# ligengen/EgoGen

Hardware: AMD Instinct MI355X
Metric: PPO env-steps/sec (512 parallel SMPL-X agents) (higher is better)
Workload: dtype f32 (blend GEMM: shape/template columns as 2-term bf16 splits, pose correctives as one fp16 product, fp32 accumulate); PPO update products on 2-term bf16 splits; rollout policy layers on 2-term bf16 splits

## Files before the change

### egogen_amd/csrc/body_model.hip

```cpp
#include <algorithm>
#include <atomic>
#include <cstdlib>

#include "lbs_pack.h"

static thread_local hipEvent_t g_prof_start = nullptr, g_prof_stop = nullptr;
extern "C" int egx_profile_next_lbs(void* start_event, void* stop_event) {
  g_prof_start = static_cast<hipEvent_t>(start_event);
  g_prof_stop = static_cast<hipEvent_t>(stop_event);
  return EGX_OK;
}

namespace {
constexpr int BODY_PAD = 256;
}

__global__ void egx_gather_kernel(const float* __restrict__ picked, int B, int NP, int M,
                                  const int* __restrict__ marker_slot, const int* __restrict__ extra_slot,
                                  const int* __restrict__ lmk_slot, const float* __restrict__ lmk_bary,
                                  float* __restrict__ out_joints, float* __restrict__ out_markers) {
  const int b = blockIdx.x;
  const float* pk = picked + (size_t)b * NP * 3;
  for (int i = threadIdx.x; i < M + NEXTRA + NLMK; i += blockDim.x) {
    if (i < M) {
      if (out_markers) {
        const float* s = pk + marker_slot[i] * 3;
        float* o = out_markers + ((size_t)b * M + i) * 3;
        o[0] = s[0]; o[1] = s[1]; o[2] = s[2];
      }
    } else if (out_joints) {
      float* o = out_joints + ((size_t)b * EGX_NUM_JOINTS_OUT + NJ + (i - M)) * 3;
      if (i < M + NEXTRA) {
        const float* s = pk + extra_slot[i - M] * 3;
        o[0] = s[0]; o[1] = s[1]; o[2] = s[2];
      } else {
        const int l = i - M - NEXTRA;
        float acc[3] = {0.f, 0.f, 0.f};
        for (int k = 0; k < 3; ++k) {
          const float* s = pk + lmk_slot[l * 3 + k] * 3;
          const float w = lmk_bary[l * 3 + k];
          acc[0] += s[0] * w; acc[1] += s[1] * w; acc[2] += s[2] * w;
        }
        o[0] = acc[0]; o[1] = acc[1]; o[2] = acc[2];
      }
    }
  }
}

extern "C" int egx_body_model_create(const egx_body_model_host* d, egx_body_model** out) {
  EGX_REQUIRE(d && out, "null argument");
  LbsPacked p;
  if (int rc = lbs_pack_model(d, &p)) return rc;
  auto* m = new egx_body_model();
  static_cast<LbsModelDims&>(*m) = p;
  auto u16 = [](bf16x8** dptr) { return reinterpret_cast<unsigned short**>(dptr); };
  int rc = EGX_OK;
  if ((rc = egx_upload(&m->cull_E, p.cull_E)) || (rc = egx_upload(&m->cull_D0, p.cull_D0)) || (rc = egx_upload(u16(&m->dirs3), p.dirs3)) ||
      (rc = egx_upload(u16(&m->dirs4), p.dirs4)) || (rc = egx_upload(u16(&m->skinW), p.skinW)) || (rc = egx_upload(&m->skin_ks_off, p.skin_ks_off)) ||
      (rc = egx_upload(&m->dirs_rm, p.dirs_rm)) || (rc = egx_upload(&m->vorig, p.perm)) || (rc = egx_upload(&m->pick_tiles, p.pick_tiles)) ||
      (rc = egx_upload(&m->sdf_tiles, p.sdf_tiles)) || (rc = egx_upload(&m->dirs, p.dirs)) || (rc = egx_upload(&m->tj_off, p.tj_off)) ||
      (rc = egx_upload(&m->tj_idx, p.tj_idx)) || (rc = egx_upload(&m->tj_w, p.tj_w)) || (rc = egx_upload(&m->pick_slot, p.pick_slot)) ||
      (rc = egx_upload(&m->vflags, p.vflags)) || (rc = egx_upload(&m->pc, p.pc)) || (rc = egx_upload(&m->marker_slot, p.marker_slot)) ||
      (rc = egx_upload(&m->extra_slot, p.extra_slot)) || (rc = egx_upload(&m->lmk_slot, p.lmk_slot)) ||
      (rc = egx_upload(&m->lmk_bary, p.lmk_bary))) {
    egx_body_model_destroy(m);
    return rc;
  }
  *out = m;
  return EGX_OK;
}

extern "C" void egx_body_model_destroy(egx_body_model* m) {
  if (!m) return;
  (void)hipFree(m->dirs); (void)hipFree(m->dirs3); (void)hipFree(m->dirs4); (void)hipFree(m->tj_off); (void)hipFree(m->tj_idx); (void)hipFree(m->tj_w);
  (void)hipFree(m->pick_slot); (void)hipFree(m->pick_tiles); (void)hipFree(m->sdf_tiles); (void)hipFree(m->vflags); (void)hipFree(m->vorig); (void)hipFree(m->pc); (void)hipFree(m->marker_slot);
  (void)hipFree(m->extra_slot); (void)hipFree(m->lmk_slot); (void)hipFree(m->lmk_bary);
  (void)hipFree(m->cull_E); (void)hipFree(m->cull_D0);
  (void)hipFree(m->skinW); (void)hipFree(m->skin_ks_off); (void)hipFree(m->dirs_rm);
  delete m;
}

extern "C" int egx_body_model_num_verts(const egx_body_model* m) { return m ? m->V : 0; }
extern "C" int egx_body_model_nnz(const egx_body_model* m) { return m ? m->NW : 0; }
extern "C" int egx_body_model_lbs_vertices(const egx_body_model* m, int with_sdf) {
  return m ? (with_sdf ? m->verts_sdf_tiles : m->verts_pick_tiles) : 0;
}

namespace {
template <typename Parse>
int switch_value(std::atomic<int>& g, const char* env_name, Parse&& parse) {
  int v = g.load();
  if (v < 0) {
    const char* e = getenv(env_name);
    v = parse(std::string(e ? e : ""));
    if (v >= 0) g.store(v);
  }
  return v;
}
std::atomic<int> g_blend_mode{-1};
int blend_mode() {
  return switch_value(g_blend_mode, "EGX_LBS_BLEND", [](const std::string& v) {
    return (v == "f32" || v == "0") ? 0 : ((v == "bf16x3" || v == "1") ? 1 : ((v == "bf16x2" || v == "2") ? 2 : ((v.empty() || v == "f16mix" || v == "3") ? 3 : -2)));
  });
}
std::atomic<int> g_cull{-1};
int culling_on() {
  return switch_value(g_cull, "EGX_LBS_CULL", [](const std::string& v) { return v == "1" ? 1 : 0; });
}
std::atomic<int> g_wave_tile{-1};
int wave_tile() {
  return switch_value(g_wave_tile, "EGX_LBS_WAVE_TILE", [](const std::string& v) { return atoi(v.c_str()); });
}
std::atomic<int> g_fixq_cap{0};

struct WsLayout {
  size_t feat, feat4, A4, picked, total;
  size_t fvec, jpos, order, flags, items, counts;
  size_t fix_e, fix_stats;
  size_t skinB, cinit;
  size_t fixq;
  size_t Bp;
  int items_stride;
};
WsLayout ws_layout(const egx_body_model* m, int B) {
  const size_t Bp = egx_align_up((size_t)B, BODY_PAD);
  WsLayout w;
  w.Bp = Bp;
// ... 253 lines not shown
```

### egogen_amd/csrc/env.hip

```cpp
#include "egx_common.h"
#include "egx_frame.h"
#include "egx_reward.h"

namespace {

constexpr int NT = 20, THIS = 2, NM = 67, NJO = EGX_NUM_JOINTS_OUT, SD = 402, XB = EGX_XB_DIM;
constexpr int NRAY = 32;
constexpr int BLK = 128;

__device__ __forceinline__ float block_reduce(float v, float* sh, int op ) {
  sh[threadIdx.x] = v;
  __syncthreads();
  for (int s = BLK / 2; s > 0; s >>= 1) {
    if ((int)threadIdx.x < s) {
      const float a = sh[threadIdx.x], b = sh[threadIdx.x + s];
      sh[threadIdx.x] = op == 0 ? a + b : (op == 1 ? fminf(a, b) : fmaxf(a, b));
    }
    __syncthreads();
  }
  const float r = sh[0];
  __syncthreads();
  return r;
}

struct SceneDev {
  const float* edges;
  const int* edge_off;
  const float* tris;
  const int* tri_off;
  const float* floor_h;
  const float* map_lin;
  int map_res;
  float* crowd_bbox;
  int crowd_G, crowd_S, crowd_k;
  float crowd_half;
  int crowd_polygon;
  int crowd_static;
};

__device__ __forceinline__ bool point_in_rings(const float* edges, int e0, int e1, double x, double y) {
  int crossings = 0;
  for (int e = e0; e < e1; ++e) {
    const float* q = edges + (size_t)e * 4;
    const double x0 = q[0], y0 = q[1], x1 = q[2], y1 = q[3];
    if ((y0 > y) != (y1 > y)) {
      const double xint = x0 + (y - y0) * (x1 - x0) / (y1 - y0);
      if (x < xint) ++crossings;
    }
  }
  return (crossings & 1) == 1;
}

__device__ __forceinline__ int scene_num_edges(const SceneDev& sc, int sc_i) {
  if (sc.crowd_bbox)
    return (sc.crowd_polygon ? sc.edge_off[1] - sc.edge_off[0] : 4) + (sc.crowd_static ? 0 : 4 * (sc.crowd_G - 1));
  return sc.edge_off[sc_i + 1] - sc.edge_off[sc_i];
}
__device__ __forceinline__ void scene_edge(const SceneDev& sc, int sc_i, int e, double& x0, double& y0, double& x1, double& y1) {
  if (!sc.crowd_bbox) {
    const float* p = sc.edges + (size_t)(sc.edge_off[sc_i] + e) * 4;
    x0 = p[0]; y0 = p[1]; x1 = p[2]; y1 = p[3];
    return;
  }
  const int n_ext = sc.crowd_polygon ? sc.edge_off[1] - sc.edge_off[0] : 4;
  if (sc.crowd_polygon && e < n_ext) {
    const float* p = sc.edges + (size_t)(sc.edge_off[0] + e) * 4;
    x0 = p[0]; y0 = p[1]; x1 = p[2]; y1 = p[3];
    return;
  }
  float lo[2], hi[2];
  int q;
  if (e < n_ext) {
    lo[0] = lo[1] = -sc.crowd_half; hi[0] = hi[1] = sc.crowd_half;
    q = e;
  } else {
    e -= n_ext - 4;
    int other = (e - 4) >> 2;
    if (other >= sc.crowd_k) ++other;
    const float* b = sc.crowd_bbox + ((size_t)other * sc.crowd_S + sc_i) * 4;
    lo[0] = b[0]; lo[1] = b[1]; hi[0] = b[2]; hi[1] = b[3];
    q = (e - 4) & 3;
  }
  const double cx[4] = {lo[0], hi[0], hi[0], lo[0]}, cy[4] = {lo[1], lo[1], hi[1], hi[1]};
  x0 = cx[q]; y0 = cy[q]; x1 = cx[(q + 1) & 3]; y1 = cy[(q + 1) & 3];
}

__device__ void egosensing_frame(const SceneDev& sc, int scene, const float* j23, const float* j24, const float* j56,
                                 const float* j57, double ray_len, float* out32 , int tid, int nthreads) {
  const float lx = j57[0] - j23[0] + j56[0] - j24[0];
  const float ly = j57[1] - j23[1] + j56[1] - j24[1];
  double la0 = (double)lx, la1 = (double)ly;
  const double ln = sqrt(la0 * la0 + la1 * la1);
  la0 /= ln; la1 /= ln;
  const float exf = (j23[0] + j24[0]) / 2.f, eyf = (j23[1] + j24[1]) / 2.f;
  const double ox = (double)exf, oy = (double)eyf;
  const int ne = scene_num_edges(sc, scene);
  int crossings = 0;
  for (int e = 0; e < ne; ++e) {
    double x0, y0, x1, y1;
    scene_edge(sc, scene, e, x0, y0, x1, y1);
    if ((y0 > oy) != (y1 > oy)) {
      const double xint = x0 + (oy - y0) * (x1 - x0) / (y1 - y0);
// ... 81 lines not shown

struct EnvCfg {
  float reproj_factor, goal_thresh, pene_thres;
  float w_skate, w_floor, w_face, w_look, w_success, w_target_dist, w_pene, w_vp;
  int max_depth, scene_kind , terminate_on_pene, pene_body;
  float ray_len;
  float vp_thresh;
  int no_goal_term;
};

struct StepArgs {
  EnvCfg cfg;
  SceneDev sc;
  int A;
  float* state;
  float* seed;
  float* R0;
  float* T0;
  float* dist;
  int* steps;
  const float* wpath;
  const int* scene_idx;
  const float* Y_gen;
  const float* pred_params;
  const float* joints;
  const float* markers_proj;
  const int* pene_count;
  const float* vp_emb;
  const int* feet_marker_idx;
  float* reward;
  int* terminated;
  float* rterms;
  int* nonfinite;
  int* invalid;
  float* obs_ego;
  float* obs_dist;
  float* obs_time;
  float* out_marker_b;
  float* out_prev_frame;
};

}

__global__ void egx_assemble_params_kernel(const float* __restrict__ seed, const float* __restrict__ Yb_gen, int A,
                                           float* __restrict__ pred_params) {
  const int idx = blockIdx.x * blockDim.x + threadIdx.x;
  if (idx >= A * XB) return;
  const int a = idx / XB, d = idx % XB;
  float* out = pred_params + (size_t)a * NT * XB + d;
  const float p0 = seed[((size_t)a * 2 + 0) * XB + d], p1 = seed[((size_t)a * 2 + 1) * XB + d];
  out[0 * XB] = p0;
  out[1 * XB] = p1;
  float g[5];
  for (int t = 0; t < 18; ++t) {
    const float v = Yb_gen[((size_t)t * A + a) * XB + d];
    if (t < 3) g[t + 2] = v;
    out[(t + 2) * XB] = v;
  }
  if (d >= 6) {
    const float b2 = (p1 + g[3]) / 2.0f;
    const float b3 = (b2 + g[4]) / 2.0f;
    out[2 * XB] = b2;
    out[3 * XB] = b3;
  }
}

__global__ __launch_bounds__(BLK) void egx_env_step_post_kernel(StepArgs p) {
  __shared__ float s_mb[NT][NM * 3];
  __shared__ float s_red[BLK];
  __shared__ float s_newseed[2][6];
  __shared__ float s_frame[24];
  __shared__ float s_scal[16];
  const int a = blockIdx.x, tid = threadIdx.x;
  const EnvCfg& c = p.cfg;
  const float* R0 = p.R0 + (size_t)a * 9;
  const float* T0 = p.T0 + (size_t)a * 3;
  float R0o[9], T0o[3];
  for (int e = 0; e < 9; ++e) R0o[e] = R0[e];
  for (int e = 0; e < 3; ++e) T0o[e] = T0[e];
  const float* J = p.joints + (size_t)a * NT * NJO * 3;
  const float* PP = p.pred_params + (size_t)a * NT * XB;
  const float wp[3] = {p.wpath[(size_t)a * 6 + 3], p.wpath[(size_t)a * 6 + 4], p.wpath[(size_t)a * 6 + 5]};

  const float rf = c.reproj_factor;
  for (int i = tid; i < NT * NM * 3; i += BLK) {
    const int t = i / (NM * 3), d = i % (NM * 3);
    const float pred = (t < THIS) ? p.state[((size_t)a * 2 + t) * SD + d] : p.Y_gen[((size_t)(t - 2) * p.A + a) * (NM * 3) + d];
    const float proj = p.markers_proj[((size_t)a * NT + t) * NM * 3 + d];
    const float v = rf * proj + (1.f - rf) * pred;
    s_mb[t][d] = v;
    if (p.out_marker_b) p.out_marker_b[((size_t)a * NT + t) * NM * 3 + d] = v;
  }
  __syncthreads();

  const auto mb_at = [&](int t, int i) { return s_mb[t][i]; };
  float part = 0.f;
  if (tid < 18) part = reward_skate_frame(mb_at, tid, p.feet_marker_idx);
  const float r_skate = expf(-(block_reduce(part, s_red, 0) / 18.f));
  part = 0.f;
  if (tid < NT) part = reward_floor_frame(R0o, T0o, mb_at, tid, p.feet_marker_idx);
  const float r_floor = expf(-(block_reduce(part, s_red, 0) / (float)NT));

  part = 0.f;
  if (tid < NT) {
    const float* e = p.vp_emb + ((size_t)a * NT + tid) * 32;
    float s = 0.f;
    for (int k = 0; k < 32; ++k) s += e[k] * e[k];
    part = sqrtf(s);
  }
  const float vp_norm = block_reduce(part, s_red, 0) / (float)NT;
  const float r_vp = (vp_norm > c.vp_thresh) ? 0.f : 0.05f;

  float r_pene = 0.f;
  bool penetration = false;
  if (c.scene_kind == 0) {
    float cs = 0.f, cm = 0.f;
    if (tid < NT) {
      cs = (float)p.pene_count[(size_t)a * NT + tid];
      cm = cs;
    }
    const float total = block_reduce(cs, s_red, 0);
    const float mx = block_reduce(cm, s_red, 2);
    r_pene = expf(-reward_pene_arg(total));
    penetration = !(mx < 40.f);
  }

  if (tid == 0) {
    const float* j19 = J + (size_t)19 * NJO * 3;
    const float* j18 = J + (size_t)18 * NJO * 3;
    float tl[3], dir[2];
    const float r_face = reward_face(j19, R0o, T0o, wp, tl, dir);
    const float f0 = dir[0], f1 = dir[1];
    float e0 = j19[24 * 3 + 0] - j19[23 * 3 + 0], e1 = j19[24 * 3 + 1] - j19[23 * 3 + 1];
    const float nrm = fmaxf(sqrtf(e0 * e0 + e1 * e1), 1e-12f);
    e0 /= nrm; e1 /= nrm;
    const float r_look = ((f0 * (-e1) + f1 * e0) + 1.f) / 2.0f;
    const float d2t = target_distance(tl, j19);
    const float r_td = p.dist[a] - d2t;
    const float r_goal = (d2t < c.goal_thresh) ? 1.f : 0.f;
    float Rn[9], Tn[3];
    canonical_frame(j18 + 0, j18 + 3, j18 + 6, Rn, Tn);
    float T0n[3], R0n[9];
    mat3_vec(R0o, Tn, T0n);
    T0n[0] += T0o[0]; T0n[1] += T0o[1]; T0n[2] += T0o[2];
    mat3_mul(R0o, Rn, R0n);
    const float delta[3] = {j18[0] - PP[18 * XB + 0], j18[1] - PP[18 * XB + 1], j18[2] - PP[18 * XB + 2]};
    update_transl_glorot(Rn, Tn, delta, PP + 18 * XB, s_newseed[0]);
    update_transl_glorot(Rn, Tn, delta, PP + 19 * XB, s_newseed[1]);
    for (int e = 0; e < 9; ++e) { s_frame[e] = Rn[e]; s_frame[12 + e] = R0n[e]; }
    for (int e = 0; e < 3; ++e) { s_frame[9 + e] = Tn[e]; s_frame[21 + e] = T0n[e]; }
    s_scal[0] = r_face; s_scal[1] = r_look; s_scal[2] = r_td; s_scal[3] = r_goal; s_scal[4] = d2t;
  }
  __syncthreads();
  float Rn[9], Tn[3], R0n[9], T0n[3];
  for (int e = 0; e < 9; ++e) { Rn[e] = s_frame[e]; R0n[e] = s_frame[12 + e]; }
  for (int e = 0; e < 3; ++e) { Tn[e] = s_frame[9 + e]; T0n[e] = s_frame[21 + e]; }
  const float r_face = s_scal[0], r_look = s_scal[1], r_td = s_scal[2], r_goal = s_scal[3], d2t = s_scal[4];

  float tln[3];
  {
    const float v[3] = {wp[0] - T0n[0], wp[1] - T0n[1], wp[2] - T0n[2]};
    mat3T_vec(R0n, v, tln);
  }
  float bminx = 3.4e38f, bminy = 3.4e38f, bmaxx = -3.4e38f, bmaxy = -3.4e38f;
  for (int i = tid; i < THIS * NM; i += BLK) {
    const int t = i / NM, m = i % NM;
    const float v[3] = {s_mb[18 + t][m * 3 + 0] - Tn[0], s_mb[18 + t][m * 3 + 1] - Tn[1], s_mb[18 + t][m * 3 + 2] - Tn[2]};
    float ms[3];
    mat3T_vec(Rn, v, ms);
    float* st = p.state + ((size_t)a * 2 + t) * SD;
    st[m * 3 + 0] = ms[0]; st[m * 3 + 1] = ms[1]; st[m * 3 + 2] = ms[2];
    marker_target_feature(tln, ms, st + 201 + m * 3);
    bool use = c.pene_body != 0;
    if (!use)
// ... 513 lines not shown
```

### egogen_amd/csrc/lbs.h

```cpp
#pragma once
#include <mutex>

#include "egx_common.h"

namespace {

constexpr int NJ = EGX_NUM_JOINTS;
constexpr int KACT = 10 + 51 * 9;
constexpr int KDIM = EGX_BLEND_K;
constexpr int KSTEPS = KDIM / 2;
constexpr int KGROUPS = KSTEPS / 4;
static_assert(KGROUPS >= 2, "the operand ring preloads two k-groups");
constexpr int KS3 = 30;
__host__ __device__ inline void egx_bf16_split3(float x, unsigned short* h) {
  h[0] = egx_bf16_rne(x);
  const float r1 = x - egx_bf16_to_f32(h[0]);
  h[1] = egx_bf16_rne(r1);
  const float r2 = r1 - egx_bf16_to_f32(h[1]);
  h[2] = egx_bf16_rne(r2);
}
constexpr int M4_BASE_PIECES = 96, M4_FEAT_PIECES = 32;
constexpr int M4_FKS = 4;
__host__ __device__ inline int egx_m4_feat_piece(int s, int pl) { return s == 0 ? pl : (s <= 28 ? s + 1 : 30 + pl); }
__host__ __device__ inline int egx_m4_base_piece(int s, int pl, int c) { return s == 0 ? pl * 3 + c : (s <= 28 ? 6 + (s - 1) * 3 + c : 90 + pl * 3 + c); }
__host__ __device__ inline unsigned short egx_f16_rne(float x) {
  const _Float16 h = (_Float16)x;
  unsigned short u;
  __builtin_memcpy(&u, &h, 2);
  return u;
}
__host__ __device__ inline int egx_compact_joint(int j) { return (j - 1) - (j > 24 ? 3 : 0); }
__host__ __device__ inline int egx_expand_joint(int jc) { return jc + 1 + (jc >= 21 ? 3 : 0); }
constexpr int NLMK = 51, NEXTRA = 21;

}

struct PoseConsts {
  int parents[NJ];
  int depth[NJ];
  int max_depth;
  float J_template[NJ * 3];
  float J_shapedirs[NJ * 3 * 10];
  float hand_comps[2 * 12 * 45];
  float hand_mean[2 * 45];
  float fix_c[NJ];
  float fix_d[NJ];
  float fix_pf;
  float fix_dpf;
  float shape_c[10];
  float vt_max;
  float w_abs_max;
};

namespace {

constexpr float LBS_FIX_SLACK_M = 3e-6f;
constexpr float LBS_TWO_PLANE_ERR = 1.2e-5f;
constexpr float LBS_ACC_ADDS_OFFSETS = 496.f;
constexpr float LBS_ACC_ADDS_LAST = 48.f;
constexpr float LBS_FIX_MARGIN = 1.001f;
constexpr float LBS_SKIN_ERR = 2.0e-5f;
constexpr int LBS_FIX_NQ = 64;
constexpr int LBS_FIX_CNT0 = 32;
constexpr int LBS_FIX_STATS_INTS = LBS_FIX_CNT0 + 32 * LBS_FIX_NQ;
constexpr int LBS_FIXQ_CAP = 1 << 12;

}

constexpr int SKIN_BT_A = NJ * 2 * 32;
constexpr int SKIN_BT_BYTES = NJ * 2 * 32 * 24;

struct LbsModelDims {
  int V = 0, NVT = 0, NW = 0, M = 0, NP = 0;
  int n_pick_tiles = 0, n_sdf_tiles = 0;
  int verts_pick_tiles = 0, verts_sdf_tiles = 0;
  int cull_ok = 0;
  int sdf_lead_picks = 0;
  float rest_pelvis[3] = {0.f, 0.f, 0.f};
  float cull_ref_margin = 0.f;
};

struct egx_body_model : LbsModelDims {
  float* dirs_rm = nullptr;
  bf16x8* skinW = nullptr;
  int* skin_ks_off = nullptr;
  f32x4* dirs = nullptr;
  bf16x8* dirs3 = nullptr;
  bf16x8* dirs4 = nullptr;
  int* tj_off = nullptr;
  int* tj_idx = nullptr;
  float* tj_w = nullptr;
  int* pick_slot = nullptr;
  int* pick_tiles = nullptr;
  int* sdf_tiles = nullptr;
  uint8_t* vflags = nullptr;
  int* vorig = nullptr;
  PoseConsts* pc = nullptr;
  int* marker_slot = nullptr;
  int* extra_slot = nullptr;
  int* lmk_slot = nullptr;
  float* lmk_bary = nullptr;
  float* cull_E = nullptr;
  float* cull_D0 = nullptr;
};

__device__ __forceinline__ void lbs_joint_rotation(const PoseConsts* __restrict__ pc, const float* __restrict__ x, int j, float (&R)[9]) {
  float a[3] = {0.f, 0.f, 0.f};
  if (j == 0) {
    a[0] = x[3]; a[1] = x[4]; a[2] = x[5];
  } else if (j <= 21) {
    a[0] = x[6 + 3 * (j - 1)]; a[1] = x[7 + 3 * (j - 1)]; a[2] = x[8 + 3 * (j - 1)];
  } else if (j >= 25) {
    const int side = (j >= 40) ? 1 : 0;
    const int o = 3 * (j - (side ? 40 : 25));
    const float* comps = pc->hand_comps + side * 12 * 45;
    const float* pca = x + 69 + side * 12;
    for (int c = 0; c < 3; ++c) {
      float s = 0.f;
      for (int k = 0; k < 12; ++k) s += pca[k] * comps[k * 45 + o + c];
      a[c] = s + pc->hand_mean[side * 45 + o + c];
    }
  }
  const float ex = a[0] + 1e-8f, ey = a[1] + 1e-8f, ez = a[2] + 1e-8f;
  const float angle = sqrtf(ex * ex + ey * ey + ez * ez);
  const float rx = a[0] / angle, ry = a[1] / angle, rz = a[2] / angle;
  const float sn = sinf(angle), cs = 1.f - cosf(angle);
  R[0] = 1.f + cs * (-(ry * ry + rz * rz)); R[1] = -sn * rz + cs * (rx * ry);     R[2] = sn * ry + cs * (rx * rz);
  R[3] = sn * rz + cs * (rx * ry);          R[4] = 1.f + cs * (-(rx * rx + rz * rz)); R[5] = -sn * rx + cs * (ry * rz);
  R[6] = -sn * ry + cs * (rx * rz);         R[7] = sn * rx + cs * (ry * rz);      R[8] = 1.f + cs * (-(rx * rx + ry * ry));
}

struct LbsParams {
  const f32x4* dirs;
  const int* tj_off;
  const int* tj_idx;
  const float* tj_w;
  const int* pick_slot;
  const int* tiles;
  int n_tiles;
  const uint8_t* vflags;
  const int* vorig;
  const bf16x8* dirs3;
  const bf16x8* feat3;
  const bf16x8* dirs4;
  const bf16x8* feat4;
  int n_precise;
  const f32x4* feat;
  const f32x4* A4;
  const float* xb;
  int B, V, NVT, NW, NP, fpa;
  int nbg;
  int bg_block;
  int dbg;
  float* verts;
  float* picked;
  SdfDev sdf;
  const float* R0;
  const float* T0;
  int* pene;
  const int* agent_of_slot;
  const int* items;
  const int* item_counts;
  int items_stride;
  const float* fix_e;
  const float* sdf_aux;
  int* fix_stats;
  const float* dirs_rm;
  const PoseConsts* pc;
  const float* betas;
  int2* fixq;
  int fixq_cap;
  const bf16x8* skinW;
  const int* skin_ks_off;
  const bf16x8* skinB;
  const f32x4* cinit;
  const SdfSceneDev* scenes;
  const int* agent_scene;
  int n_scenes;
};

__device__ __forceinline__ bool lbs_scene_of(const LbsParams& p, int ag, int& s) {
  const int v = p.agent_scene[ag];
  const bool ok = v >= 0 && v < p.n_scenes;
  s = ok ? v : 0;
  return ok;
}

__device__ __forceinline__ int lbs_live_slot(int bt, int n, int B) { return min(bt * 32 + n, B - 1); }

__device__ __forceinline__ float lbs_fma(float a, float b, float c) {
  float d;
  asm("v_fma_f32 %0, %1, %2, %3" : "=v"(d) : "v"(a), "v"(b), "v"(c));
  return d;
}

struct LbsWave {
  int lane, n, half;
  float* s_W;
  int* s_jl;
  int* s_slot;
  unsigned* s_masks;
  int* s_cnt;
  unsigned* s_fixmap;
  float* s_thr;
  float* lds;
  f32x4* s_queue;
  int qn;
#ifdef EGX_LBS_TIMING
  unsigned long long et[8] = {0, 0, 0, 0, 0, 0, 0, 0};
#endif
};
constexpr int LBS_NB = 2;
// ... 62 lines not shown
```

### egogen_amd/csrc/lbs_epilogue.h

```cpp
#pragma once
#include "lbs.h"

constexpr int LBS_META_BYTES = 7680;
constexpr int LBS_VERT_BYTES = 32 * 97 * 4;
constexpr int LBS_QCAP = 640;
constexpr int LBS_THREADS = 512;

template <bool WRITE_VERTS, bool DO_SDF>
__device__ __forceinline__ LbsWave lbs_wave_init(char* my, int lane) {
  LbsWave w;
  w.lane = lane; w.n = lane & 31; w.half = lane >> 5;
  w.s_W = reinterpret_cast<float*>(my);
  w.s_jl = reinterpret_cast<int*>(my + NJ * 32 * 4);
  w.s_slot = w.s_jl + 56;
  w.s_masks = reinterpret_cast<unsigned*>(w.s_slot + 32);
  w.s_cnt = reinterpret_cast<int*>(w.s_masks + 4);
  w.lds = reinterpret_cast<float*>(my + LBS_META_BYTES);
  w.s_queue = reinterpret_cast<f32x4*>(my + LBS_META_BYTES);
  w.s_fixmap = nullptr; w.s_thr = nullptr;
  w.qn = 0;
  w.s_cnt[lane] = 0;
  return w;
}

__device__ __forceinline__ int lbs_load_meta(const LbsParams& p, LbsWave& w, int vt) {
  const int lane = w.lane;
  float* s_W = w.s_W; int* s_jl = w.s_jl; int* s_slot = w.s_slot; unsigned* s_masks = w.s_masks;
  const int j_lo = p.tj_off[vt];
  const int JT = p.tj_off[vt + 1] - j_lo;
  for (int idx = lane * 4; idx < JT * 32; idx += 256)
    *reinterpret_cast<f32x4*>(&s_W[idx]) = *reinterpret_cast<const f32x4*>(&p.tj_w[(size_t)j_lo * 32 + idx]);
  if (lane < JT) s_jl[lane] = p.tj_idx[j_lo + lane];
  {
    const int sl = (lane < 32) ? p.pick_slot[vt * 32 + lane] : -1;
    const int fl = (lane < 32) ? p.vflags[vt * 32 + lane] : 0;
    if (lane < 32) s_slot[lane] = sl;
    const unsigned long long mp = __ballot(sl >= 0), ms = __ballot((fl & 3) == 2);
    if (lane == 0) { s_masks[0] = (unsigned)mp; s_masks[1] = (unsigned)ms; }
  }
  __builtin_amdgcn_wave_barrier();

  return JT;
}

__device__ __forceinline__ void lbs_fix_blend_planes(const LbsParams& p, int lane, int vt, int row, int bt, int n, float (&v)[3]) {
  v[0] = v[1] = v[2] = 0.f;
  if (lane < 2 * KS3) {
    const int sidx = lane >> 1, hf = lane & 1;
    float f[8];
#pragma unroll
    for (int e = 0; e < 8; ++e) f[e] = 0.f;
#pragma unroll
    for (int pl = 2; pl >= 0; --pl) {
      const bf16x8 fr = p.feat3[(((size_t)bt * KS3 + sidx) * 3 + pl) * 64 + hf * 32 + n];
#pragma unroll
      for (int e = 0; e < 8; ++e) f[e] += egx_bf16_to_f32((unsigned short)fr[e]);
    }
    if (sidx == KS3 - 1 && hf == 0) f[6] = 0.f;
#pragma unroll
    for (int c = 0; c < 3; ++c) {
      float b[8];
#pragma unroll
      for (int e = 0; e < 8; ++e) b[e] = 0.f;
#pragma unroll
      for (int pl = 2; pl >= 0; --pl) {
        const bf16x8 br = p.dirs3[((((size_t)vt * KS3 + sidx) * 3 + pl) * 3 + c) * 64 + hf * 32 + row];
#pragma unroll
        for (int e = 0; e < 8; ++e) b[e] += egx_bf16_to_f32((unsigned short)br[e]);
      }
#pragma unroll
      for (int e = 0; e < 8; ++e) v[c] = fmaf(f[e], b[e], v[c]);
    }
  }
}

template <bool VERTEX_MAJOR, bool MS = false>
__device__ __forceinline__ float lbs_fix_one(const LbsParams& p, int lane, int vt, int row, int slot, int JT, const int* jl, const float* Wt) {
  const int bt = slot >> 5, n = slot & 31;
  const int body = p.agent_of_slot ? p.agent_of_slot[slot / p.fpa] * p.fpa + slot % p.fpa : slot;
  const int ag = body / p.fpa;
  SdfDev sd = p.sdf;
  if constexpr (MS) {
    int sc;
    lbs_scene_of(p, ag, sc);
    sd = egx_sdf_scene(p.sdf, p.scenes[sc]);
  }
  float v[3] = {0.f, 0.f, 0.f};
  if constexpr (!VERTEX_MAJOR) {
    lbs_fix_blend_planes(p, lane, vt, row, bt, n, v);
  } else {
    const float* x = p.xb + (size_t)body * EGX_XB_DIM;
    const float* base = p.dirs_rm + ((size_t)vt * 32 + row) * 3 * KDIM;
    if (lane == 0) {
      const float* be = p.betas + (size_t)ag * 10;
#pragma unroll
      for (int c = 0; c < 3; ++c) {
        float acc = base[c * KDIM + KACT];
        for (int k = 0; k < 10; ++k) acc = fmaf(be[k], base[c * KDIM + k], acc);
        v[c] = acc;
      }
    } else if (lane < NJ && (lane < 22 || lane > 24)) {
      float R[9];
      lbs_joint_rotation(p.pc, x, lane, R);
      const int k0 = 10 + egx_compact_joint(lane) * 9;
#pragma unroll
      for (int c = 0; c < 3; ++c) {
        float acc = 0.f;
#pragma unroll
        for (int e = 0; e < 9; ++e) acc = fmaf(R[e] - ((e == 0 || e == 4 || e == 8) ? 1.f : 0.f), base[c * KDIM + k0 + e], acc);
        v[c] = acc;
      }
    }
  }
#pragma unroll
  for (int c = 0; c < 3; ++c) v[c] = lbs_wave_sum(v[c]);
  float o[3] = {0.f, 0.f, 0.f};
  if (lane < JT) {
    const int j = jl[lane] & 0xff;
    const float wv = Wt[lane * 32 + row];
    const f32x4* Aq = p.A4 + ((size_t)bt * NJ + j) * 3 * 32 + n;
#pragma unroll
    for (int a = 0; a < 3; ++a) {
      const f32x4 ar = Aq[a * 32];
      o[a] = wv * fmaf(ar[0], v[0], fmaf(ar[1], v[1], fmaf(ar[2], v[2], ar[3])));
    }
  }
#pragma unroll
  for (int a = 0; a < 3; ++a) o[a] = lbs_wave_sum(o[a]) + p.xb[(size_t)body * EGX_XB_DIM + a];
  const float kk[3] = {sd.scale * (float)sd.d0 * 0.5f, sd.scale * (float)sd.d1 * 0.5f, sd.scale * (float)sd.d2 * 0.5f};
  const float cc[3] = {sd.cx, sd.cy, sd.cz};
  const float dd[3] = {(float)sd.d0, (float)sd.d1, (float)sd.d2};
  float vox[3];
#pragma unroll
  for (int a = 0; a < 3; ++a) {
    float Mw[3];
#pragma unroll
    for (int e = 0; e < 3; ++e) Mw[e] = kk[a] * (p.R0 ? p.R0[(size_t)ag * 9 + a * 3 + e] : ((a == e) ? 1.f : 0.f));
    const float tw = kk[a] * ((p.T0 ? p.T0[(size_t)ag * 3 + a] : 0.f) - cc[a]) + (dd[a] - 1.f) * 0.5f;
    vox[a] = fmaf(Mw[0], o[0], fmaf(Mw[1], o[1], fmaf(Mw[2], o[2], tw)));
  }
  return egx_sdf_neg_trilinear_at(sd, __builtin_amdgcn_fmed3f(vox[0], 0.f, (float)(sd.d0 - 1)), __builtin_amdgcn_fmed3f(vox[1], 0.f, (float)(sd.d1 - 1)),
                                  __builtin_amdgcn_fmed3f(vox[2], 0.f, (float)(sd.d2 - 1)));
}

template <int NB, bool MS = false>
__device__ __forceinline__ void lbs_fix_process(const LbsParams& p, const LbsWave& w, int vt, int bt0, int JT) {
  const int lane = w.lane;
  unsigned mybits = lane < 32 * NB ? w.s_fixmap[lane] : 0u;
  if (mybits != 0u) w.s_fixmap[lane] = 0u;
  unsigned long long pend = __ballot(mybits != 0u);
  const int mine = __popc(mybits);
  int total = 0, my_off = 0;
  for (unsigned long long m = pend; m != 0ull; m &= m - 1) {
    const int sl = __builtin_ctzll(m);
    if (lane == sl) my_off = total;
    total += __builtin_amdgcn_readlane(mine, sl);
  }
  int base = 0;
  const int sq = blockIdx.x % LBS_FIX_NQ;
  int2* q = p.fixq + (size_t)sq * p.fixq_cap;
  if (lane == 0) base = atomicAdd(p.fix_stats + LBS_FIX_CNT0 + 32 * sq, total);
  base = __builtin_amdgcn_readfirstlane(base);
  if (base + total <= p.fixq_cap) {
    const int slot = min((bt0 + (lane >> 5)) * 32 + (lane & 31), p.B - 1);
    for (int k = 0; mybits != 0u; ++k) {
      const int row = __builtin_ctz(mybits);
      mybits &= mybits - 1;
      q[base + my_off + k] = make_int2(vt * 32 + row, slot);
    }
    return;
  }
  for (int i = base + lane; i < min(base + total, p.fixq_cap); i += 64) q[i] = make_int2(-1, 0);
  while (pend != 0ull) {
    const int sl = __builtin_ctzll(pend);
    pend &= pend - 1;
    unsigned bits = (unsigned)__builtin_amdgcn_readlane((int)mybits, sl);
    const int slot = min((bt0 + (sl >> 5)) * 32 + (sl & 31), p.B - 1);
    while (bits != 0u) {
      const int row = __builtin_ctz(bits);
      bits &= bits - 1;
      const float sv = lbs_fix_one<false, MS>(p, lane, vt, row, slot, JT, w.s_jl, w.s_W);
      if (lane == 0) {
        if (sv < 0.f) atomicAdd(&w.s_cnt[sl], 1);
        atomicAdd(p.fix_stats, 1);
      }
    }
  }
}

template <bool WRITE_VERTS, bool DO_SDF, int RB, int QCAP, int NB = LBS_NB, bool FIX = false, bool MS = false>
__device__ __forceinline__ void lbs_epilogue(const LbsParams& p, LbsWave& w, f32x16 (&acc)[3][NB], int vt, int bt0, int JT, bool fix_on = false) {
  const int lane = w.lane, n = w.n, half = w.half;
  float* s_W = w.s_W; int* s_jl = w.s_jl; int* s_slot = w.s_slot; unsigned* s_masks = w.s_masks; int* s_cnt = w.s_cnt;
  float* lds = w.lds; f32x4* s_queue = w.s_queue;
  int qn = w.qn;
  float tr[NB][3];
  int body[NB];
  bool bvalid[NB];
#pragma unroll
  for (int q = 0; q < NB; ++q) {
    const int slot = (bt0 + q) * 32 + n;
    bvalid[q] = slot < p.B;
    const int sl = bvalid[q] ? slot : p.B - 1;
    body[q] = p.agent_of_slot ? p.agent_of_slot[sl / p.fpa] * p.fpa + sl % p.fpa : sl;
    const int bb = body[q];
    tr[q][0] = p.xb[(size_t)bb * EGX_XB_DIM + 0];
    tr[q][1] = p.xb[(size_t)bb * EGX_XB_DIM + 1];
    tr[q][2] = p.xb[(size_t)bb * EGX_XB_DIM + 2];
  }
  [[maybe_unused]] float thr[NB];
#pragma unroll
  for (int q = 0; q < NB; ++q) thr[q] = 0.f;
  if constexpr (FIX && DO_SDF && !MS) {
    if (fix_on) {
      const float lip = p.sdf_aux[3];
#pragma unroll
      for (int q = 0; q < NB; ++q) {
        thr[q] = p.fix_e[min((bt0 + q) * 32 + n, p.B - 1)] * lip;
        w.s_thr[q * 32 + n] = thr[q];
      }
    }
  }
  auto sdf_flush = [&](int count) {
    __builtin_amdgcn_wave_barrier();
    for (int base = 0; base < count; base += 64) {
      const int idx = base + lane;
      if (idx < count) {
        const f32x4 e = s_queue[idx];
        int code = __float_as_int(e[3]);
        float sv;
        if constexpr (MS) {
          sv = egx_sdf_neg_trilinear_at(egx_sdf_scene(p.sdf, p.scenes[code >> 16]), e[0], e[1], e[2]);
          code &= 0xffff;
        } else {
          sv = egx_sdf_neg_trilinear_at(p.sdf, e[0], e[1], e[2]);
        }
        if constexpr (FIX) {
          const float t = fix_on ? w.s_thr[code & 63] : 0.f;
          if (sv < -t) atomicAdd(&s_cnt[code & 63], 1);
          else if (fix_on && sv <= t) {
            const int rr = (code >> 8) & 15;
            atomicOr(&w.s_fixmap[code & 63], 1u << ((rr & 3) + 8 * (rr >> 2) + 4 * (code >> 12)));
          }
        } else {
          if (sv < 0.f) atomicAdd(&s_cnt[code & 63], 1);
        }
      }
    }
    __builtin_amdgcn_wave_barrier();
  };
  const unsigned pick_mask = p.picked ? (unsigned)__builtin_amdgcn_readfirstlane((int)s_masks[0]) : 0u;
  const unsigned sdf_mask = (unsigned)__builtin_amdgcn_readfirstlane((int)s_masks[1]);
#ifdef EGX_LBS_TIMING
  unsigned long long (&et)[8] = w.et;
#endif
#pragma unroll
  for (int q = 0; q < NB; ++q) {
    [[maybe_unused]] const unsigned long long q0 = LBS_NOW();
    const int ls = lbs_live_slot(bt0 + q, n, p.B);
    const f32x4* Aq = p.A4 + (size_t)(ls >> 5) * NJ * 3 * 32 + (ls & 31);
    float o[16][3];
#pragma unroll
    for (int r = 0; r < 16; ++r) { o[r][0] = tr[q][0]; o[r][1] = tr[q][1]; o[r][2] = tr[q][2]; }
    f32x4 a0, a1, a2;
// ... 184 lines not shown
```

### egogen_amd/csrc/lbs_fix.hip

```cpp
#include "lbs_epilogue.h"

constexpr int LBS_FIX_BLOCKS = 1024;
static_assert((LBS_FIX_BLOCKS * 4) % LBS_FIX_NQ == 0, "waves of the fix-up kernel per sub-queue");
template <bool MS>
__global__ __launch_bounds__(256) void egx_lbs_fix_kernel(LbsParams p) {
  const int lane = threadIdx.x & 63;
  const int wave = blockIdx.x * 4 + (threadIdx.x >> 6), n_waves = gridDim.x * 4;
  const int sq = wave % LBS_FIX_NQ;
  const int count = min(p.fix_stats[LBS_FIX_CNT0 + 32 * sq], p.fixq_cap);
  for (int i = wave / LBS_FIX_NQ; i < count; i += n_waves / LBS_FIX_NQ) {
    const int2 e = p.fixq[(size_t)sq * p.fixq_cap + i];
    if (e.x < 0) continue;
    const int vt = e.x >> 5, row = e.x & 31, slot = e.y;
    const int j_lo = p.tj_off[vt], JT = p.tj_off[vt + 1] - j_lo;
    const float sv = lbs_fix_one<true, MS>(p, lane, vt, row, slot, JT, p.tj_idx + j_lo, p.tj_w + (size_t)j_lo * 32);
    if (lane == 0 && sv < 0.f) {
      const int body = p.agent_of_slot ? p.agent_of_slot[slot / p.fpa] * p.fpa + slot % p.fpa : slot;
      atomicAdd(p.pene + body, 1);
    }
  }
}

void lbs_launch_fix(const LbsParams& p, bool ms, hipStream_t stream) {
  hipLaunchKernelGGL(ms ? egx_lbs_fix_kernel<true> : egx_lbs_fix_kernel<false>, dim3(LBS_FIX_BLOCKS), dim3(256), 0, stream, p);
}
```

Measured before the change: 193,800.

## Software-pipeline LBS fix-up queue, restructure reductions and marker blend loads

```diff
diff --git a/egogen_amd/csrc/body_model.hip b/egogen_amd/csrc/body_model.hip
--- a/egogen_amd/csrc/body_model.hip
+++ b/egogen_amd/csrc/body_model.hip
@@ -19,30 +19,31 @@
                                   const int* __restrict__ marker_slot, const int* __restrict__ extra_slot,
                                   const int* __restrict__ lmk_slot, const float* __restrict__ lmk_bary,
                                   float* __restrict__ out_joints, float* __restrict__ out_markers) {
+#pragma clang fp contract(off)
   const int b = blockIdx.x;
   const float* pk = picked + (size_t)b * NP * 3;
   for (int i = threadIdx.x; i < M + NEXTRA + NLMK; i += blockDim.x) {
-    if (i < M) {
-      if (out_markers) {
-        const float* s = pk + marker_slot[i] * 3;
-        float* o = out_markers + ((size_t)b * M + i) * 3;
-        o[0] = s[0]; o[1] = s[1]; o[2] = s[2];
-      }
-    } else if (out_joints) {
-      float* o = out_joints + ((size_t)b * EGX_NUM_JOINTS_OUT + NJ + (i - M)) * 3;
-      if (i < M + NEXTRA) {
-        const float* s = pk + extra_slot[i - M] * 3;
-        o[0] = s[0]; o[1] = s[1]; o[2] = s[2];
-      } else {
-        const int l = i - M - NEXTRA;
-        float acc[3] = {0.f, 0.f, 0.f};
-        for (int k = 0; k < 3; ++k) {
-          const float* s = pk + lmk_slot[l * 3 + k] * 3;
-          const float w = lmk_bary[l * 3 + k];
-          acc[0] += s[0] * w; acc[1] += s[1] * w; acc[2] += s[2] * w;
-        }
-        o[0] = acc[0]; o[1] = acc[1]; o[2] = acc[2];
-      }
+    const bool marker = i < M, lmk = i >= M + NEXTRA;
+    if (marker ? !out_markers : !out_joints) continue;
+    const int l = lmk ? i - M - NEXTRA : 0;
+    const int* first = marker ? marker_slot + i : (lmk ? lmk_slot + l * 3 : extra_slot + (i - M));
+    int sl[3];
+    float w[3];
+    sl[0] = first[0]; sl[1] = lmk_slot[l * 3 + 1]; sl[2] = lmk_slot[l * 3 + 2];
+#pragma unroll
+    for (int k = 0; k < 3; ++k) w[k] = lmk_bary[l * 3 + k];
+    float s[3][3];
+#pragma unroll
+    for (int k = 0; k < 3; ++k)
+#pragma unroll
+      for (int c = 0; c < 3; ++c) s[k][c] = pk[sl[k] * 3 + c];
+    float* o = marker ? out_markers + ((size_t)b * M + i) * 3 : out_joints + ((size_t)b * EGX_NUM_JOINTS_OUT + NJ + (i - M)) * 3;
+    if (lmk) {
+      o[0] = fmaf(s[2][0], w[2], fmaf(s[1][0], w[1], fmaf(s[0][0], w[0], 0.f)));
+      o[1] = fmaf(s[2][1], w[2], fmaf(s[1][1], w[1], fmaf(s[0][1], w[0], 0.f)));
+      o[2] = ((0.f + s[0][2] * w[0]) + s[1][2] * w[1]) + s[2][2] * w[2];
+    } else {
+      o[0] = s[0][0]; o[1] = s[0][1]; o[2] = s[0][2];
     }
   }
 }
diff --git a/egogen_amd/csrc/egx_reduce.h b/egogen_amd/csrc/egx_reduce.h
--- /dev/null
+++ b/egogen_amd/csrc/egx_reduce.h
@@ -0,0 +1,28 @@
+#pragma once
+#include <cmath>
+
+#if defined(__HIPCC__) || defined(__CUDACC__)
+#define EGX_REDUCE_HD __host__ __device__
+#else
+#define EGX_REDUCE_HD
+#endif
+
+EGX_REDUCE_HD inline float egx_reduce_op(float a, float b, int op ) {
+  return op == 0 ? a + b : (op == 1 ? fminf(a, b) : fmaxf(a, b));
+}
+
+template <class Holder>
+EGX_REDUCE_HD inline void egx_reduce_tree128(Holder& h, int op) {
+  h.fold_upper_half(op);
+  for (int s = 32; s > 0; s >>= 1) h.fold_lane_above(s, op);
+}
+
+struct EgxReduceHost128 {
+  float v[128];
+  void fold_upper_half(int op) {
+    for (int i = 0; i < 64; ++i) v[i] = egx_reduce_op(v[i], v[i + 64], op);
+  }
+  void fold_lane_above(int s, int op) {
+    for (int i = 0; i < 64; ++i) v[i] = egx_reduce_op(v[i], i + s < 64 ? v[i + s] : v[i], op);
+  }
+};
diff --git a/egogen_amd/csrc/env.hip b/egogen_amd/csrc/env.hip
--- a/egogen_amd/csrc/env.hip
+++ b/egogen_amd/csrc/env.hip
@@ -1,5 +1,6 @@
 #include "egx_common.h"
 #include "egx_frame.h"
+#include "egx_reduce.h"
 #include "egx_reward.h"
 
 namespace {
@@ -8,16 +9,23 @@
 constexpr int NRAY = 32;
 constexpr int BLK = 128;
 
+struct BlockReduceLane {
+  float x;
+  const float* sh;
+  __device__ __forceinline__ void fold_upper_half(int op) { x = egx_reduce_op(sh[threadIdx.x], sh[threadIdx.x + 64], op); }
+  __device__ __forceinline__ void fold_lane_above(int s, int op) { x = egx_reduce_op(x, __shfl_down(x, s), op); }
+};
+
 __device__ __forceinline__ float block_reduce(float v, float* sh, int op ) {
+  static_assert(BLK == 128, "egx_reduce_tree128");
   sh[threadIdx.x] = v;
   __syncthreads();
-  for (int s = BLK / 2; s > 0; s >>= 1) {
-    if ((int)threadIdx.x < s) {
-      const float a = sh[threadIdx.x], b = sh[threadIdx.x + s];
-      sh[threadIdx.x] = op == 0 ? a + b : (op == 1 ? fminf(a, b) : fmaxf(a, b));
-    }
-    __syncthreads();
-  }
+  if (threadIdx.x < 64) {
+    BlockReduceLane l{0.f, sh};
+    egx_reduce_tree128(l, op);
+    if (threadIdx.x == 0) sh[0] = l.x;
+  }
+  __syncthreads();
   const float r = sh[0];
   __syncthreads();
   return r;
@@ -265,14 +273,23 @@
   const float* PP = p.pred_params + (size_t)a * NT * XB;
   const float wp[3] = {p.wpath[(size_t)a * 6 + 3], p.wpath[(size_t)a * 6 + 4], p.wpath[(size_t)a * 6 + 5]};
 
-  const float rf = c.reproj_factor;
-  for (int i = tid; i < NT * NM * 3; i += BLK) {
-    const int t = i / (NM * 3), d = i % (NM * 3);
-    const float pred = (t < THIS) ? p.state[((size_t)a * 2 + t) * SD + d] : p.Y_gen[((size_t)(t - 2) * p.A + a) * (NM * 3) + d];
-    const float proj = p.markers_proj[((size_t)a * NT + t) * NM * 3 + d];
-    const float v = rf * proj + (1.f - rf) * pred;
-    s_mb[t][d] = v;
-    if (p.out_marker_b) p.out_marker_b[((size_t)a * NT + t) * NM * 3 + d] = v;
+  const float rf = c.reproj_factor, rf1 = 1.f - rf;
+  for (int d = tid; d < NM * 3; d += BLK) {
+    float pred[NT], proj[NT];
+#pragma unroll
+    for (int t = 0; t < NT; ++t) {
+      pred[t] = (t < THIS) ? p.state[((size_t)a * 2 + t) * SD + d] : p.Y_gen[((size_t)(t - 2) * p.A + a) * (NM * 3) + d];
+      proj[t] = p.markers_proj[((size_t)a * NT + t) * NM * 3 + d];
+    }
+#pragma unroll
+    for (int t = 0; t < NT; ++t) {
+      pred[t] = fmaf(rf1, pred[t], rf * proj[t]);
+      s_mb[t][d] = pred[t];
+    }
+    if (p.out_marker_b) {
+#pragma unroll
+      for (int t = 0; t < NT; ++t) p.out_marker_b[((size_t)a * NT + t) * NM * 3 + d] = pred[t];
+    }
   }
   __syncthreads();
 
diff --git a/egogen_amd/csrc/lbs.h b/egogen_amd/csrc/lbs.h
--- a/egogen_amd/csrc/lbs.h
+++ b/egogen_amd/csrc/lbs.h
@@ -104,30 +104,46 @@
   float* cull_D0 = nullptr;
 };
 
-__device__ __forceinline__ void lbs_joint_rotation(const PoseConsts* __restrict__ pc, const float* __restrict__ x, int j, float (&R)[9]) {
-  float a[3] = {0.f, 0.f, 0.f};
-  if (j == 0) {
-    a[0] = x[3]; a[1] = x[4]; a[2] = x[5];
-  } else if (j <= 21) {
-    a[0] = x[6 + 3 * (j - 1)]; a[1] = x[7 + 3 * (j - 1)]; a[2] = x[8 + 3 * (j - 1)];
-  } else if (j >= 25) {
-    const int side = (j >= 40) ? 1 : 0;
-    const int o = 3 * (j - (side ? 40 : 25));
-    const float* comps = pc->hand_comps + side * 12 * 45;
-    const float* pca = x + 69 + side * 12;
-    for (int c = 0; c < 3; ++c) {
-      float s = 0.f;
-      for (int k = 0; k < 12; ++k) s += pca[k] * comps[k * 45 + o + c];
-      a[c] = s + pc->hand_mean[side * 45 + o + c];
-    }
+struct LbsJointIn {
+  float m[3];
+  float pk[12];
+  float cm[12][3];
+};
+__device__ __forceinline__ void lbs_joint_request(const PoseConsts* __restrict__ pc, const float* __restrict__ x, int j, LbsJointIn& in) {
+  const bool hand = j >= 25 && j < NJ;
+  const int side = (hand && j >= 40) ? 1 : 0;
+  const int o = hand ? 3 * (j - (side ? 40 : 25)) : 0;
+  const float* m = hand ? pc->hand_mean + side * 45 + o : x + 3 + 3 * (j <= 21 ? j : 0);
+  const float* comps = pc->hand_comps + side * 12 * 45 + o;
+  const float* pca = x + 69 + side * 12;
+#pragma unroll
+  for (int c = 0; c < 3; ++c) in.m[c] = m[c];
+#pragma unroll
+  for (int k = 0; k < 12; ++k) {
+    in.pk[k] = pca[k];
+#pragma unroll
+    for (int c = 0; c < 3; ++c) in.cm[k][c] = comps[k * 45 + c];
+  }
+}
+__device__ __forceinline__ void lbs_joint_rotation(const LbsJointIn& in, int j, float (&R)[9]) {
+#pragma clang fp contract(off)
+  float a[3];
+#pragma unroll
+  for (int c = 0; c < 3; ++c) {
+    float s = 0.f;
+#pragma unroll
+    for (int k = 0; k < 12; ++k) s = (c < 2 || k < 2) ? fmaf(in.pk[k], in.cm[k][c], s) : s + in.pk[k] * in.cm[k][c];
+    a[c] = (j >= 25 && j < NJ) ? s + in.m[c] : (j <= 21 ? in.m[c] : 0.f);
   }
   const float ex = a[0] + 1e-8f, ey = a[1] + 1e-8f, ez = a[2] + 1e-8f;
-  const float angle = sqrtf(ex * ex + ey * ey + ez * ez);
+  const float angle = sqrtf(ez * ez + fmaf(ey, ey, ex * ex));
   const float rx = a[0] / angle, ry = a[1] / angle, rz = a[2] / angle;
   const float sn = sinf(angle), cs = 1.f - cosf(angle);
-  R[0] = 1.f + cs * (-(ry * ry + rz * rz)); R[1] = -sn * rz + cs * (rx * ry);     R[2] = sn * ry + cs * (rx * rz);
-  R[3] = sn * rz + cs * (rx * ry);          R[4] = 1.f + cs * (-(rx * rx + rz * rz)); R[5] = -sn * rx + cs * (ry * rz);
-  R[6] = -sn * ry + cs * (rx * rz);         R[7] = sn * rx + cs * (ry * rz);      R[8] = 1.f + cs * (-(rx * rx + ry * ry));
+  const float xx = rx * rx, yy = ry * ry, xz = rx * rz;
+  const float cxy = (rx * ry) * cs, cyz = (ry * rz) * cs, sy = ry * sn;
+  R[0] = fmaf(-fmaf(rz, rz, yy), cs, 1.f); R[1] = fmaf(-rz, sn, cxy);               R[2] = fmaf(xz, cs, sy);
+  R[3] = fmaf(rz, sn, cxy);                R[4] = fmaf(-fmaf(rz, rz, xx), cs, 1.f); R[5] = fmaf(-rx, sn, cyz);
+  R[6] = fmaf(xz, cs, -sy);                R[7] = fmaf(rx, sn, cyz);                R[8] = fmaf(-(xx + yy), cs, 1.f);
 }
 
 struct LbsParams {
diff --git a/egogen_amd/csrc/lbs_epilogue.h b/egogen_amd/csrc/lbs_epilogue.h
--- a/egogen_amd/csrc/lbs_epilogue.h
+++ b/egogen_amd/csrc/lbs_epilogue.h
@@ -74,7 +74,7 @@
   }
 }
 
-template <bool VERTEX_MAJOR, bool MS = false>
+template <bool MS = false>
 __device__ __forceinline__ float lbs_fix_one(const LbsParams& p, int lane, int vt, int row, int slot, int JT, const int* jl, const float* Wt) {
   const int bt = slot >> 5, n = slot & 31;
   const int body = p.agent_of_slot ? p.agent_of_slot[slot / p.fpa] * p.fpa + slot % p.fpa : slot;
@@ -86,32 +86,7 @@
     sd = egx_sdf_scene(p.sdf, p.scenes[sc]);
   }
   float v[3] = {0.f, 0.f, 0.f};
-  if constexpr (!VERTEX_MAJOR) {
-    lbs_fix_blend_planes(p, lane, vt, row, bt, n, v);
-  } else {
-    const float* x = p.xb + (size_t)body * EGX_XB_DIM;
-    const float* base = p.dirs_rm + ((size_t)vt * 32 + row) * 3 * KDIM;
-    if (lane == 0) {
-      const float* be = p.betas + (size_t)ag * 10;
-#pragma unroll
-      for (int c = 0; c < 3; ++c) {
-        float acc = base[c * KDIM + KACT];
-        for (int k = 0; k < 10; ++k) acc = fmaf(be[k], base[c * KDIM + k], acc);
-        v[c] = acc;
-      }
-    } else if (lane < NJ && (lane < 22 || lane > 24)) {
-      float R[9];
-      lbs_joint_rotation(p.pc, x, lane, R);
-      const int k0 = 10 + egx_compact_joint(lane) * 9;
-#pragma unroll
-      for (int c = 0; c < 3; ++c) {
-        float acc = 0.f;
-#pragma unroll
-        for (int e = 0; e < 9; ++e) acc = fmaf(R[e] - ((e == 0 || e == 4 || e == 8) ? 1.f : 0.f), base[c * KDIM + k0 + e], acc);
-        v[c] = acc;
-      }
-    }
-  }
+  lbs_fix_blend_planes(p, lane, vt, row, bt, n, v);
 #pragma unroll
   for (int c = 0; c < 3; ++c) v[c] = lbs_wave_sum(v[c]);
   float o[3] = {0.f, 0.f, 0.f};
@@ -179,7 +154,7 @@
     while (bits != 0u) {
       const int row = __builtin_ctz(bits);
       bits &= bits - 1;
-      const float sv = lbs_fix_one<false, MS>(p, lane, vt, row, slot, JT, w.s_jl, w.s_W);
+      const float sv = lbs_fix_one<MS>(p, lane, vt, row, slot, JT, w.s_jl, w.s_W);
       if (lane == 0) {
         if (sv < 0.f) atomicAdd(&w.s_cnt[sl], 1);
         atomicAdd(p.fix_stats, 1);
diff --git a/egogen_amd/csrc/lbs_fix.hip b/egogen_amd/csrc/lbs_fix.hip
--- a/egogen_amd/csrc/lbs_fix.hip
+++ b/egogen_amd/csrc/lbs_fix.hip
@@ -1,23 +1,153 @@
 #include "lbs_epilogue.h"
 
-constexpr int LBS_FIX_BLOCKS = 1024;
+namespace {
+
+struct FixHead {
+  int vt, row, slot;
+  bool live;
+  int tj0, tj1, aos;
+};
+struct FixLink {
+  int jl, scene;
+};
+__device__ __forceinline__ int lbs_fix_j_lo(const FixHead& h) { return __builtin_amdgcn_readfirstlane(h.tj0); }
+__device__ __forceinline__ int lbs_fix_jt(const FixHead& h) { return __builtin_amdgcn_readfirstlane(h.tj1 - h.tj0); }
+__device__ __forceinline__ int lbs_fix_body(const LbsParams& p, const FixHead& h) {
+  return p.agent_of_slot ? __builtin_amdgcn_readfirstlane(h.aos) * p.fpa + h.slot % p.fpa : h.slot;
+}
+
+__device__ __forceinline__ int2 lbs_fix_record(const LbsParams& p, int sq, int i, int count) {
+  return p.fixq[(size_t)sq * p.fixq_cap + min(i, count - 1)];
+}
+
+__device__ __forceinline__ FixHead lbs_fix_head(const LbsParams& p, int2 rec, bool in_range) {
+  const int ex = __builtin_amdgcn_readfirstlane(rec.x), ey = __builtin_amdgcn_readfirstlane(rec.y);
+  FixHead h;
+  h.live = in_range && ex >= 0;
+  const int code = h.live ? ex : 0;
+  h.vt = code >> 5; h.row = code & 31; h.slot = h.live ? ey : 0;
+  h.tj0 = p.tj_off[h.vt];
+  h.tj1 = p.tj_off[h.vt + 1];
+  h.aos = p.agent_of_slot ? p.agent_of_slot[h.slot / p.fpa] : 0;
+  return h;
+}
+
+template <bool MS>
+__device__ __forceinline__ FixLink lbs_fix_link(const LbsParams& p, int lane, const FixHead& h) {
+  FixLink l;
+  l.jl = p.tj_idx[lbs_fix_j_lo(h) + min(lane, max(lbs_fix_jt(h), 1) - 1)];
+  l.scene = 0;
+  if constexpr (MS) l.scene = p.agent_scene[lbs_fix_body(p, h) / p.fpa];
+  return l;
+}
+
+template <bool MS>
+__device__ __forceinline__ float lbs_fix_vertex(const LbsParams& p, int lane, const FixHead& h, const FixLink& l) {
+  const int bt = h.slot >> 5, n = h.slot & 31, row = h.row;
+  const int j_lo = lbs_fix_j_lo(h), JT = lbs_fix_jt(h);
+  const int body = lbs_fix_body(p, h);
+  const int ag = body / p.fpa;
+  const float* x = p.xb + (size_t)body * EGX_XB_DIM;
+  const float* base = p.dirs_rm + ((size_t)h.vt * 32 + row) * 3 * KDIM;
+  const int jj = min(lane, max(JT, 1) - 1);
+  const f32x4* Aq = p.A4 + ((size_t)bt * NJ + (l.jl & 0xff)) * 3 * 32 + n;
+  const float wv = p.tj_w[(size_t)(j_lo + jj) * 32 + row];
+  f32x4 ar[3];
+#pragma unroll
+  for (int a = 0; a < 3; ++a) ar[a] = Aq[a * 32];
+  SdfDev sd = p.sdf;
+  if constexpr (MS) {
+    const bool ok = l.scene >= 0 && l.scene < p.n_scenes;
+    sd = egx_sdf_scene(p.sdf, p.scenes[ok ? l.scene : 0]);
+  }
+  constexpr int U_R0 = 0, U_T0 = 9, U_TR = 12, U_BE = 15, U_END = 25;
+  float uni;
+  {
+    const float* src = x;
+    if (lane < U_T0) { if (p.R0) src = p.R0 + (size_t)ag * 9 + lane; }
+    else if (lane < U_TR) { if (p.T0) src = p.T0 + (size_t)ag * 3 + (lane - U_T0); }
+    else if (lane < U_BE) src = x + (lane - U_TR);
+    else if (lane < U_END) src = p.betas + (size_t)ag * 10 + (lane - U_BE);
+    uni = *src;
+  }
+  const auto uniform = [&](int k) { return __int_as_float(__builtin_amdgcn_readlane(__float_as_int(uni), k)); };
+  const bool shape_lane = lane == 0, pose_lane = lane > 0 && lane < NJ && (lane < 22 || lane > 24);
+  const int k0 = pose_lane ? 10 + egx_compact_joint(lane) * 9 : 0;
+  float bv[3][9], b9[3], tpl[3];
+#pragma unroll
+  for (int c = 0; c < 3; ++c) {
+#pragma unroll
+    for (int e = 0; e < 9; ++e) bv[c][e] = base[c * KDIM + k0 + e];
+    b9[c] = base[c * KDIM + 9];
+    tpl[c] = base[c * KDIM + KACT];
+  }
+  LbsJointIn rin;
+  lbs_joint_request(p.pc, x, lane, rin);
+  __builtin_amdgcn_sched_barrier(0);
+  float R[9];
+  lbs_joint_rotation(rin, lane, R);
+  float v[3];
+#pragma unroll
+  for (int c = 0; c < 3; ++c) {
+    float sh = tpl[c];
+#pragma unroll
+    for (int k = 0; k < 10; ++k) sh = fmaf(uniform(U_BE + k), k < 9 ? bv[c][k] : b9[c], sh);
+    float po = 0.f;
+#pragma unroll
+    for (int e = 0; e < 9; ++e) po = fmaf(R[e] - ((e == 0 || e == 4 || e == 8) ? 1.f : 0.f), bv[c][e], po);
+    v[c] = shape_lane ? sh : (pose_lane ? po : 0.f);
+  }
+#pragma unroll
+  for (int c = 0; c < 3; ++c) v[c] = lbs_wave_sum(v[c]);
+  float o[3] = {0.f, 0.f, 0.f};
+  if (lane < JT) {
+#pragma unroll
+    for (int a = 0; a < 3; ++a) o[a] = wv * fmaf(ar[a][0], v[0], fmaf(ar[a][1], v[1], fmaf(ar[a][2], v[2], ar[a][3])));
+  }
+#pragma unroll
+  for (int a = 0; a < 3; ++a) o[a] = lbs_wave_sum(o[a]) + uniform(U_TR + a);
+  const float kk[3] = {sd.scale * (float)sd.d0 * 0.5f, sd.scale * (float)sd.d1 * 0.5f, sd.scale * (float)sd.d2 * 0.5f};
+  const float cc[3] = {sd.cx, sd.cy, sd.cz};
+  const float dd[3] = {(float)sd.d0, (float)sd.d1, (float)sd.d2};
+  float vox[3];
+#pragma unroll
+  for (int a = 0; a < 3; ++a) {
+    float Mw[3];
+#pragma unroll
+    for (int e = 0; e < 3; ++e) Mw[e] = kk[a] * (p.R0 ? uniform(U_R0 + a * 3 + e) : ((a == e) ? 1.f : 0.f));
+    const float tw = kk[a] * ((p.T0 ? uniform(U_T0 + a) : 0.f) - cc[a]) + (dd[a] - 1.f) * 0.5f;
+    vox[a] = fmaf(Mw[0], o[0], fmaf(Mw[1], o[1], fmaf(Mw[2], o[2], tw)));
+  }
+  return egx_sdf_neg_trilinear_at(sd, __builtin_amdgcn_fmed3f(vox[0], 0.f, (float)(sd.d0 - 1)), __builtin_amdgcn_fmed3f(vox[1], 0.f, (float)(sd.d1 - 1)),
+                                  __builtin_amdgcn_fmed3f(vox[2], 0.f, (float)(sd.d2 - 1)));
+}
+
+}
+
+constexpr int LBS_FIX_BLOCKS = 768;
 static_assert((LBS_FIX_BLOCKS * 4) % LBS_FIX_NQ == 0, "waves of the fix-up kernel per sub-queue");
 template <bool MS>
 __global__ __launch_bounds__(256) void egx_lbs_fix_kernel(LbsParams p) {
   const int lane = threadIdx.x & 63;
-  const int wave = blockIdx.x * 4 + (threadIdx.x >> 6), n_waves = gridDim.x * 4;
+  const int wave = blockIdx.x * 4 + __builtin_amdgcn_readfirstlane(threadIdx.x >> 6), n_waves = gridDim.x * 4;
   const int sq = wave % LBS_FIX_NQ;
-  const int count = min(p.fix_stats[LBS_FIX_CNT0 + 32 * sq], p.fixq_cap);
-  for (int i = wave / LBS_FIX_NQ; i < count; i += n_waves / LBS_FIX_NQ) {
-    const int2 e = p.fixq[(size_t)sq * p.fixq_cap + i];
-    if (e.x < 0) continue;
-    const int vt = e.x >> 5, row = e.x & 31, slot = e.y;
-    const int j_lo = p.tj_off[vt], JT = p.tj_off[vt + 1] - j_lo;
-    const float sv = lbs_fix_one<true, MS>(p, lane, vt, row, slot, JT, p.tj_idx + j_lo, p.tj_w + (size_t)j_lo * 32);
-    if (lane == 0 && sv < 0.f) {
-      const int body = p.agent_of_slot ? p.agent_of_slot[slot / p.fpa] * p.fpa + slot % p.fpa : slot;
-      atomicAdd(p.pene + body, 1);
+  const int step = n_waves / LBS_FIX_NQ;
+  const int count = min(__builtin_amdgcn_readfirstlane(p.fix_stats[LBS_FIX_CNT0 + 32 * sq]), p.fixq_cap);
+  int i = wave / LBS_FIX_NQ;
+  if (i >= count) return;
+  FixHead h = lbs_fix_head(p, lbs_fix_record(p, sq, i, count), true);
+  FixHead h1 = lbs_fix_head(p, lbs_fix_record(p, sq, i + step, count), i + step < count);
+  int2 e2 = lbs_fix_record(p, sq, i + 2 * step, count);
+  FixLink l = lbs_fix_link<MS>(p, lane, h);
+  for (; i < count; i += step) {
+    const int2 e3 = lbs_fix_record(p, sq, i + 3 * step, count);
+    const FixHead h2 = lbs_fix_head(p, e2, i + 2 * step < count);
+    const FixLink l1 = lbs_fix_link<MS>(p, lane, h1);
+    if (h.live) {
+      const float sv = lbs_fix_vertex<MS>(p, lane, h, l);
+      if (lane == 0 && sv < 0.f) atomicAdd(p.pene + lbs_fix_body(p, h), 1);
     }
+    h = h1; h1 = h2; l = l1; e2 = e3;
   }
 }
 
```

Result: no change. 195,600, median of 6 (+0.9%).
